# vlongle/pixie

Hardware: AMD Instinct MI355X
Metric: voxels/s (128^3 U-Net fwd) + MPM particle-steps/s (higher is better)
Workload: dtype f32 (operands split fp16 hi+lo, 3 f16 MFMAs/product, fp32 accumulate); 1 GPU; 128^3x64 feature grid -> SegmentationUNet+RegressionUNet forward (+argmax/one-hot combine), 1 scene per GPU per step; grid=128, feature_channels=64, parallelism=scene-parallel x1, executor=c+hip_graph

## Files before the change

### pixie_amd/csrc/conv3d_f16x3.hip

```cpp
#include <hip/hip_runtime.h>

#include <cstdlib>
#include <map>
#include <string>
#include <type_traits>

#include "../../include/pixie_hip.h"
#include "common.h"
#include "conv_plan.h"

namespace pixie {

typedef float f32x16 __attribute__((ext_vector_type(16)));
typedef _Float16 f16x8 __attribute__((ext_vector_type(8)));

constexpr int kW16HeaderU4 = 4;

struct Conv16Args {
    const float* in0; const float* in1;
    int c0, cin;
    int ID, IH, IW;
    int LD, LH, LW;
    int ups;
    int stride;
    int OD, OH, OW;
    const float* pro_a; const float* pro_b; const float* gamma; const float* beta;
    int act;
    const uint4* w16;
    const float* wf;
    const float* bias;
    int cout, coutp;
    const float* residual; float* out;
    const unsigned* amax0; const unsigned* amax1;
    float in_bound;
    int TX, TY, TZ, lTX, lTY;
    int tiles_x, tiles_y, tiles_z, n_tiles;
    int HX, HY, HZ, HYX, CS;
    unsigned mHX, mHYX;
    float* stats; unsigned* out_amax;
    float* partial; int chunks_per_slice;
    int epi_lds;
    const float* sk_in0; const float* sk_in1;
    int sk_c0, sk_cin;
    const uint4* sk_w16; const float* sk_bias;
    const unsigned* sk_amax0; const unsigned* sk_amax1;
};

__device__ __forceinline__ int fast_div16(int n, int d, unsigned magic) {
    return (d == 1) ? n : (int)__umulhi((unsigned)n, magic);
}
__device__ __forceinline__ float act16(float t, int act) {
    if (act == 1) return t > 0.0f ? t : 0.02f * t;
    if (act == 2) return t / (1.0f + __expf(-t));
    return t;
}
__device__ __forceinline__ float act16_staged(float t, int act) {
    if (act == 1) return fmaxf(t, 0.02f * t);
    if (act == 2) return t / (1.0f + __expf(-t));
    return t;
}
__device__ __forceinline__ int scale_exponent(float bound) {
    const unsigned bits = __float_as_uint(bound);
    const int eb = (int)((bits >> 23) & 0xffu) - 127;
    if (!(bound > 0.0f) || eb > 100) return 0;
    int e = 14 - eb;
    return e > 100 ? 100 : (e < -100 ? -100 : e);
}
__device__ __forceinline__ float pow2i(int e) { return __uint_as_float((unsigned)(e + 127) << 23); }

template <int KS, int MB, int NB, bool EX = false, bool SP = false, int SK = 0, bool PAIR = false>
__device__ __forceinline__ void conv3d_f16x3_body(const Conv16Args& A) {
    static_assert(!PAIR || (MB == 2 && !EX && !SP && SK == 0), "pair form: the plain f16x3 body with 64 c_out per quartet");
    static_assert(!SP || (KS == 3 && NB == 4 && !EX), "sub-pixel path: 3^3, two x parities x two voxel blocks per wave");
    static_assert(SK == 0 || (!EX && !SP), "folded skip (SK: 1 register-fed, 2 staged through LDS): f16x3, no sub-pixel form");
    extern __shared__ uint4 smem16[];
    constexpr int PAD = (KS == 3) ? 1 : 0;
    constexpr int NW = 4, NT = 64 * NW;
    const int bufsz = 4 * A.CS;

    const int tid = threadIdx.x;
    const int lane = tid & 63;
    const int quartet = PAIR ? __builtin_amdgcn_readfirstlane(tid >> 8) : 0;
    const int wave = PAIR ? (tid >> 6) & 3 : tid >> 6;
    const int qtid = PAIR ? tid & 255 : tid;
    const int kh = lane >> 5;
    const int l31 = lane & 31;

    int t = blockIdx.x;
    {
        const int per = (A.n_tiles + 7) >> 3;
        const int cand = (t & 7) * per + (t >> 3);
        if ((A.n_tiles & 7) == 0) t = cand;
    }
    int par = 0;
    if constexpr (SP) { par = t & 3; t >>= 2; }
    const int py = par & 1, pz = par >> 1;
    const int tx = t % A.tiles_x; t /= A.tiles_x;
    const int ty = t % A.tiles_y;
    const int tz = t / A.tiles_y;
    const int ox0 = tx * A.TX, oy0 = ty * A.TY, oz0 = tz * A.TZ;
    const int cout0 = (PAIR ? 2 * (int)blockIdx.y + quartet : (int)blockIdx.y) * (MB * 32);
    const int lx0 = SP ? ox0 - 1 : ox0 * A.stride - PAD;
    const int ly0 = SP ? oy0 - 1 + py : oy0 * A.stride - PAD;
    const int lz0 = SP ? oz0 - 1 + pz : oz0 * A.stride - PAD;
    const size_t ISP = (size_t)A.ID * A.IH * A.IW;
    const size_t OSP = (size_t)A.OD * A.OH * A.OW;

    int voff[NB];
    int ovox[NB];
    bool valid[NB];
#pragma unroll
    for (int nb = 0; nb < NB; ++nb) {
        if constexpr (SP) {
            const int px = nb >> 1;
            const int j = (wave * 2 + (nb & 1)) * 32 + l31;
            int x = j & (A.TX - 1);
            int y = (j >> A.lTX) & (A.TY - 1);
            int z = j >> (A.lTX + A.lTY);
            const int gx = 2 * (ox0 + x) + px, gy = 2 * (oy0 + y) + py, gz = 2 * (oz0 + z) + pz;
            const bool v = (z < A.TZ) && (gx < A.OW) && (gy < A.OH) && (gz < A.OD);
            if (!v) { x = 0; y = 0; z = 0; }
            voff[nb] = (z * A.HY + y) * A.HX + x + px + kh * A.CS;
            ovox[nb] = v ? (gz * A.OH + gy) * A.OW + gx : 0;
            valid[nb] = v;
            continue;
        }
        const int j = (wave * NB + nb) * 32 + l31;
        int x = j & (A.TX - 1);
        int y = (j >> A.lTX) & (A.TY - 1);
        int z = j >> (A.lTX + A.lTY);
        const bool v = (z < A.TZ) && (ox0 + x < A.OW) && (oy0 + y < A.OH) && (oz0 + z < A.OD);
        if (!v) { x = 0; y = 0; z = 0; }
        voff[nb] = ((z * A.HY + y) * A.HX + x) * A.stride + kh * A.CS;
        ovox[nb] = ((oz0 + z) * A.OH + (oy0 + y)) * A.OW + ox0 + x;
        valid[nb] = v;
    }

    float bound = A.in_bound;
    if (A.amax0) {
        bound = __uint_as_float(*A.amax0);
        if (A.amax1) bound = fmaxf(bound, __uint_as_float(*A.amax1));
    }
    const int ex = EX ? 0 : scale_exponent(bound);
    const float sx = pow2i(ex);

    f32x16 acc[MB][NB];
#pragma unroll
    for (int mb = 0; mb < MB; ++mb)
#pragma unroll
        for (int nb = 0; nb < NB; ++nb)
#pragma unroll
            for (int r = 0; r < 16; ++r) acc[mb][nb][r] = 0.0f;

    const int KG = A.cin >> 3;
    const size_t tap_stride = (size_t)KG * A.coutp;
    const size_t plane = (size_t)(SP ? 64 : KS * KS * KS) * tap_stride;
    const uint4* wHi = A.w16 + kW16HeaderU4 + (size_t)kh * A.coutp + cout0 + l31 + (size_t)(par * 16) * tap_stride;
    const uint4* wLo = wHi + plane;
    const float* wF = A.wf + (size_t)kh * A.coutp + cout0 + l31;

    constexpr int TAPS = KS * KS * KS;
    auto stage_chunk = [&](int c_base, uint4* buf, int stid, int nthr, int s0, int s1) {
        uint4* bHi = buf;
        uint4* bLo = buf + 2 * A.CS;
        float pa[16], pb[16];
        {
            float pv = 0.0f;
            if (A.pro_a) pv = (lane & 16) ? A.pro_b[c_base + (lane & 15)] : A.pro_a[c_base + (lane & 15)];
#pragma unroll
            for (int j = 0; j < 16; ++j) {
                pa[j] = __int_as_float(__builtin_amdgcn_readlane(__float_as_int(pv), j));
                pb[j] = __int_as_float(__builtin_amdgcn_readlane(__float_as_int(pv), 16 + j));
            }
        }
        const bool has_aff = A.gamma != nullptr;
        using T = std::true_type; using F = std::false_type;
        if constexpr (EX) {
            float* bF = reinterpret_cast<float*>(buf);
            for (int v0 = stid; v0 < A.CS; v0 += 2 * nthr) {
                float val[2][16];
                float gm[2], bt[2];
                int sidx[2];
                bool ok[2];
#pragma unroll
                for (int u = 0; u < 2; ++u) {
                    const int vox = v0 + u * nthr;
                    int rem = vox;
                    const int hz = fast_div16(rem, A.HYX, A.mHYX);
                    rem -= hz * A.HYX;
                    const int hy = fast_div16(rem, A.HX, A.mHX);
                    const int hx = rem - hy * A.HX;
                    const int lz = lz0 + hz, ly = ly0 + hy, lx = lx0 + hx;
                    ok[u] = vox < A.CS && (unsigned)lz < (unsigned)A.LD && (unsigned)ly < (unsigned)A.LH && (unsigned)lx < (unsigned)A.LW;
                    sidx[u] = ok[u] ? ((lz >> A.ups) * A.IH + (ly >> A.ups)) * A.IW + (lx >> A.ups) : 0;
                }
#pragma unroll
                for (int u = 0; u < 2; ++u) {
#pragma unroll
                    for (int j = 0; j < 16; ++j) {
                        const int cg = c_base + j;
                        const float* src = (cg < A.c0) ? (A.in0 + (size_t)cg * ISP) : (A.in1 + (size_t)(cg - A.c0) * ISP);
                        val[u][j] = src[sidx[u]];
                    }
                    gm[u] = 1.0f; bt[u] = 0.0f;
                    if (has_aff) { gm[u] = A.gamma[sidx[u]]; bt[u] = A.beta[sidx[u]]; }
// ... 185 lines not shown
        const uint4* ldsLo = buf + 2 * A.CS;
        const uint4* wh = wHi + (size_t)(c_base >> 3) * A.coutp;
        const uint4* wl = wLo + (size_t)(c_base >> 3) * A.coutp;
        if constexpr (SP) {
            f16x8 ah[MB], al[MB];
#pragma unroll
            for (int mb = 0; mb < MB; ++mb) {
                ah[mb] = __builtin_bit_cast(f16x8, wh[mb * 32]);
                al[mb] = __builtin_bit_cast(f16x8, wl[mb * 32]);
            }
#pragma unroll 1
            for (int zy = 0; zy < 4; ++zy) {
                const int rowoff = ((zy >> 1) * A.HY + (zy & 1)) * A.HX;
                const int zyn = zy < 3 ? zy + 1 : 3;
#pragma unroll
                for (int q = 0; q < 4; ++q) {
                    const int ex = q >> 1, px = q & 1;
                    const size_t nxt = (q < 3) ? (size_t)(((q + 1) & 1) * 8 + zy * 2 + ((q + 1) >> 1)) * tap_stride : (size_t)(zyn * 2) * tap_stride;
                    f16x8 ahn[MB], aln[MB];
#pragma unroll
                    for (int mb = 0; mb < MB; ++mb) {
                        ahn[mb] = __builtin_bit_cast(f16x8, wh[nxt + mb * 32]);
                        aln[mb] = __builtin_bit_cast(f16x8, wl[nxt + mb * 32]);
                    }
                    __builtin_amdgcn_sched_barrier(0);
                    f16x8 bh[2], bl[2];
#pragma unroll
                    for (int s = 0; s < 2; ++s) {
                        bh[s] = __builtin_bit_cast(f16x8, ldsHi[voff[px * 2 + s] + rowoff + ex]);
                        bl[s] = __builtin_bit_cast(f16x8, ldsLo[voff[px * 2 + s] + rowoff + ex]);
                    }
#pragma unroll
                    for (int mb = 0; mb < MB; ++mb)
#pragma unroll
                        for (int s = 0; s < 2; ++s)
                            acc[mb][px * 2 + s] = __builtin_amdgcn_mfma_f32_32x32x16_f16(al[mb], bh[s], acc[mb][px * 2 + s], 0, 0, 0);
#pragma unroll
                    for (int mb = 0; mb < MB; ++mb)
#pragma unroll
                        for (int s = 0; s < 2; ++s)
                            acc[mb][px * 2 + s] = __builtin_amdgcn_mfma_f32_32x32x16_f16(ah[mb], bl[s], acc[mb][px * 2 + s], 0, 0, 0);
#pragma unroll
                    for (int mb = 0; mb < MB; ++mb)
#pragma unroll
                        for (int s = 0; s < 2; ++s)
                            acc[mb][px * 2 + s] = __builtin_amdgcn_mfma_f32_32x32x16_f16(ah[mb], bh[s], acc[mb][px * 2 + s], 0, 0, 0);
#pragma unroll
                    for (int mb = 0; mb < MB; ++mb) { ah[mb] = ahn[mb]; al[mb] = aln[mb]; }
                }
            }
            __builtin_amdgcn_s_setprio(0);
            return;
        }
        f16x8 ah[MB], al[MB];
#pragma unroll
        for (int mb = 0; mb < MB; ++mb) {
            ah[mb] = __builtin_bit_cast(f16x8, wh[mb * 32]);
            al[mb] = __builtin_bit_cast(f16x8, wl[mb * 32]);
        }
#pragma unroll 1
        for (int zy = 0; zy < KS * KS; ++zy) {
            const int dz = zy / KS, dy = zy - dz * KS;
            const int rowoff = (dz * A.HY + dy) * A.HX;
#pragma unroll
            for (int dx = 0; dx < KS; ++dx) {
                const int tap = zy * KS + dx;
                const int nxt = (tap + 1 < TAPS) ? tap + 1 : tap;
                f16x8 ahn[MB], aln[MB];
#pragma unroll
                for (int mb = 0; mb < MB; ++mb) {
                    ahn[mb] = __builtin_bit_cast(f16x8, wh[(size_t)nxt * tap_stride + mb * 32]);
                    aln[mb] = __builtin_bit_cast(f16x8, wl[(size_t)nxt * tap_stride + mb * 32]);
                }
                __builtin_amdgcn_sched_barrier(0);
                f16x8 bh[NB], bl[NB];
#pragma unroll
                for (int nb = 0; nb < NB; ++nb) {
                    bh[nb] = __builtin_bit_cast(f16x8, ldsHi[voff[nb] + rowoff + dx]);
                    bl[nb] = __builtin_bit_cast(f16x8, ldsLo[voff[nb] + rowoff + dx]);
                }
#pragma unroll
                for (int mb = 0; mb < MB; ++mb)
#pragma unroll
                    for (int nb = 0; nb < NB; ++nb)
                        acc[mb][nb] = __builtin_amdgcn_mfma_f32_32x32x16_f16(al[mb], bh[nb], acc[mb][nb], 0, 0, 0);
#pragma unroll
                for (int mb = 0; mb < MB; ++mb)
#pragma unroll
                    for (int nb = 0; nb < NB; ++nb)
                        acc[mb][nb] = __builtin_amdgcn_mfma_f32_32x32x16_f16(ah[mb], bl[nb], acc[mb][nb], 0, 0, 0);
#pragma unroll
                for (int mb = 0; mb < MB; ++mb)
#pragma unroll
                    for (int nb = 0; nb < NB; ++nb)
                        acc[mb][nb] = __builtin_amdgcn_mfma_f32_32x32x16_f16(ah[mb], bh[nb], acc[mb][nb], 0, 0, 0);
#pragma unroll
                for (int mb = 0; mb < MB; ++mb) { ah[mb] = ahn[mb]; al[mb] = aln[mb]; }
            }
        }
        __builtin_amdgcn_s_setprio(0);
    };

    float inv2 = 0.0f;
    {
        const int c_begin = A.partial ? (int)blockIdx.z * A.chunks_per_slice * 16 : 0;
        const int c_end = A.partial ? min(A.cin, c_begin + A.chunks_per_slice * 16) : A.cin;
        if constexpr (PAIR) {
            const int n_chunks = (c_end - c_begin) >> 4;
            const int half = (A.CS + 1) >> 1;
            const int s0 = quartet ? half : 0, s1 = quartet ? A.CS : half;
#pragma unroll 1
            for (int h = -1; h < 2 * n_chunks; ++h) {
                const int k = h >> 1;
                const bool stage = (h < 0 || ((h + quartet) & 1) == 0) && k + 1 < n_chunks;
                const bool multiply = h >= 0 && ((h + quartet) & 1) != 0;
                if (stage) stage_chunk(c_begin + 16 * (k + 1), smem16 + ((k + 1) & 1) * bufsz, qtid, NT, s0, s1);
                if (multiply) mfma_chunk(c_begin + 16 * k, smem16 + (k & 1) * bufsz);
                if (h & 1) __syncthreads();
            }
        } else {
        for (int c_base = c_begin; c_base < c_end; c_base += 16) {
            __syncthreads();
            stage_chunk(c_base, smem16, tid, NT, 0, A.CS);
            __syncthreads();
            mfma_chunk(c_base, smem16);
        }
        }
        if constexpr (SK != 0) {
            float sb = __uint_as_float(*A.sk_amax0);
            if (A.sk_amax1) sb = fmaxf(sb, __uint_as_float(*A.sk_amax1));
            const int ex2 = scale_exponent(sb);
            const float sx2 = pow2i(ex2);
            const float inv_main = __uint_as_float(A.w16[0].x) * pow2i(-ex);
            inv2 = __uint_as_float(A.sk_w16[0].x) * pow2i(-ex2);
            const float ratio = inv_main / inv2;
#pragma unroll
            for (int mb = 0; mb < MB; ++mb)
#pragma unroll
                for (int nb = 0; nb < NB; ++nb)
#pragma unroll
                    for (int r = 0; r < 16; ++r) acc[mb][nb][r] *= ratio;
            auto sk_chunks = [&]() {
                int l31s = l31, khs = kh, waves = wave;
                asm volatile("" : "+v"(l31s), "+v"(khs), "+v"(waves));
                const unsigned chb = 4u * (unsigned)ISP;
                unsigned off[NB];
#pragma unroll
                for (int nb = 0; nb < NB; ++nb) {
                    const int j = (waves * NB + nb) * 32 + l31s;
                    const int x = j & (A.TX - 1), y = (j >> A.lTX) & (A.TY - 1), z = j >> (A.lTX + A.lTY);
                    off[nb] = (valid[nb] ? 4u * (unsigned)(((oz0 + z) * A.IH + (oy0 + y)) * A.IW + ox0 + x) : 0u) + 8u * (unsigned)khs * chb;
// ... 68 lines not shown
                        const bool okv = (ox0 + x < A.OW) && (oy0 + y < A.OH) && (oz0 + z < A.OD);
                        const size_t sidx = okv ? ((size_t)(oz0 + z) * A.IH + (oy0 + y)) * A.IW + ox0 + x : 0;
                        float val[16];
#pragma unroll
                        for (int q = 0; q < 16; ++q) {
                            const int cg = c2 + q;
                            const float* src = (cg < A.sk_c0) ? (A.sk_in0 + (size_t)cg * ISP) : (A.sk_in1 + (size_t)(cg - A.sk_c0) * ISP);
                            val[q] = src[sidx];
                        }
                        f16x8 vh[2], vl[2];
#pragma unroll
                        for (int q = 0; q < 16; ++q) {
                            const float sc = okv ? val[q] * sx2 : 0.0f;
                            const _Float16 hq = (_Float16)sc;
                            vh[q >> 3][q & 7] = hq;
                            vl[q >> 3][q & 7] = (_Float16)(sc - (float)hq);
                        }
                        const int slot = (z * A.HY + y) * A.HX + x + centre;
                        bHi[slot] = __builtin_bit_cast(uint4, vh[0]);
                        bHi[A.CS + slot] = __builtin_bit_cast(uint4, vh[1]);
                        bLo[slot] = __builtin_bit_cast(uint4, vl[0]);
                        bLo[A.CS + slot] = __builtin_bit_cast(uint4, vl[1]);
                    }
                    __syncthreads();
                    f16x8 bh[NB], bl[NB];
#pragma unroll
                    for (int nb = 0; nb < NB; ++nb) {
                        bh[nb] = __builtin_bit_cast(f16x8, bHi[voff[nb] + centre]);
                        bl[nb] = __builtin_bit_cast(f16x8, bLo[voff[nb] + centre]);
                    }
#pragma unroll
                    for (int mb = 0; mb < MB; ++mb)
#pragma unroll
                        for (int nb = 0; nb < NB; ++nb)
                            acc[mb][nb] = __builtin_amdgcn_mfma_f32_32x32x16_f16(al[mb], bh[nb], acc[mb][nb], 0, 0, 0);
#pragma unroll
                    for (int mb = 0; mb < MB; ++mb)
#pragma unroll
                        for (int nb = 0; nb < NB; ++nb)
                            acc[mb][nb] = __builtin_amdgcn_mfma_f32_32x32x16_f16(ah[mb], bl[nb], acc[mb][nb], 0, 0, 0);
#pragma unroll
                    for (int mb = 0; mb < MB; ++mb)
#pragma unroll
                        for (int nb = 0; nb < NB; ++nb)
                            acc[mb][nb] = __builtin_amdgcn_mfma_f32_32x32x16_f16(ah[mb], bh[nb], acc[mb][nb], 0, 0, 0);
                }
            } else {
                sk_chunks();
            }
        }
    }

    const float inv = EX ? 1.0f : (SK != 0 ? inv2 : __uint_as_float(A.w16[0].x) * pow2i(-ex));
    if (A.partial) {
        float* dst = A.partial + (size_t)blockIdx.z * A.cout * OSP;
#pragma unroll
        for (int mb = 0; mb < MB; ++mb)
#pragma unroll
            for (int r = 0; r < 16; ++r) {
                const int co = cout0 + mb * 32 + (r & 3) + 8 * (r >> 2) + 4 * kh;
                if (co < A.cout) {
#pragma unroll
                    for (int nb = 0; nb < NB; ++nb)
                        if (valid[nb]) dst[(size_t)co * OSP + ovox[nb]] = acc[mb][nb][r] * inv;
                }
            }
        return;
    }
    constexpr int LDO_ = NB * 32 + 4;
    float* red = reinterpret_cast<float*>(smem16) + (PAIR ? (A.epi_lds ? 2 * NW * 32 * LDO_ : 0) + quartet * (NW * MB * 64) : 0);
    float wmax = 0.0f;
    const bool full = SP ? (A.epi_lds && cout0 + MB * 32 <= A.cout && (A.TX & 1) == 0 && (A.OW & 3) == 0 && NW * 64 <= A.TX * A.TY * A.TZ &&
                            2 * (ox0 + A.TX) <= A.OW && 2 * (oy0 + A.TY) <= A.OH && 2 * (oz0 + A.TZ) <= A.OD)
                         : (A.epi_lds && cout0 + MB * 32 <= A.cout && (A.TX & 3) == 0 && (A.OW & 3) == 0 && NW * NB * 32 <= A.TX * A.TY * A.TZ &&
                            ox0 + A.TX <= A.OW && oy0 + A.TY <= A.OH && oz0 + A.TZ <= A.OD);
    if (full) {
        constexpr int LDO = NB * 32 + 4;
        float* ldsO = reinterpret_cast<float*>(smem16) + (quartet * NW + wave) * (32 * LDO);
        if constexpr (!PAIR) red = reinterpret_cast<float*>(smem16) + NW * 32 * LDO;
        constexpr int LPR = NB * 8;
        constexpr int RPI = 32 / LPR;
        constexpr int NIT = 16 / RPI;
        constexpr int G = 4;
        constexpr int GPB = NIT / G;
        constexpr int NGRP = MB * GPB;
        const int rsub = l31 / LPR, colq = 4 * (l31 % LPR), nbq = colq >> 5;
        const float* nobias = EX ? A.wf : reinterpret_cast<const float*>(A.w16);
        const bool hb0 = A.bias != nullptr, hb1 = A.sk_bias != nullptr;
        float braw[MB][2];
#pragma unroll
        for (int mb = 0; mb < MB; ++mb) {
            braw[mb][0] = (hb0 ? A.bias : nobias)[cout0 + mb * 32 + l31];
            braw[mb][1] = (hb1 ? A.sk_bias : nobias)[cout0 + mb * 32 + l31];
        }
        __syncthreads();
        const int jq = SP ? wave * 64 + (colq >> 1) : (wave * NB + nbq) * 32 + (colq & 31);
        const int xq = jq & (A.TX - 1), yq = (jq >> A.lTX) & (A.TY - 1), zq = jq >> (A.lTX + A.lTY);
        const size_t ovq = SP ? ((size_t)(2 * (oz0 + zq) + pz) * A.OH + (2 * (oy0 + yq) + py)) * A.OW + 2 * (ox0 + xq)
                              : ((size_t)(oz0 + zq) * A.OH + (oy0 + yq)) * A.OW + ox0 + xq;
        const size_t orow0 = (size_t)(cout0 + kh * RPI + rsub) * OSP + ovq;
        auto rows = [&](auto res_c, auto stats_c) {
            constexpr bool RES = decltype(res_c)::value, STATS = decltype(stats_c)::value;
            size_t step = (size_t)(2 * RPI) * OSP;
            asm volatile("" : "+s"(step));
            const float* pr = A.residual + orow0;
            float* po = A.out + orow0;
            float4 r4[2][G];
            auto fetch = [&](int q) {
#pragma unroll
                for (int g = 0; g < G; ++g) { r4[q & 1][g] = *reinterpret_cast<const float4*>(pr); pr += step; }
            };
#pragma unroll
            for (int q = 0; q < NGRP; ++q) {
                const int mb = q / GPB, it0 = (q % GPB) * G;
                asm volatile("" ::: "memory");
                if (q % GPB == 0) {
                    const int brow = __float_as_int((hb0 ? braw[mb][0] : 0.0f) + (hb1 ? braw[mb][1] : 0.0f));
#pragma unroll
                    for (int r = 0; r < 16; ++r) {
                        const int row = (r & 3) + 8 * (r >> 2);
                        const int blo = __builtin_amdgcn_readlane(brow, row), bhi = __builtin_amdgcn_readlane(brow, row + 4);
                        const float bv = __int_as_float(kh ? bhi : blo);
#pragma unroll
                        for (int nb = 0; nb < NB; ++nb)
                            ldsO[((r & 3) + 8 * (r >> 2) + 4 * kh) * LDO + (SP ? 2 * ((nb & 1) * 32 + l31) + (nb >> 1) : nb * 32 + l31)] =
                                __builtin_fmaf(acc[mb][nb][r], inv, bv);
                    }
                }
                if constexpr (RES) {
                    if (q == 0) fetch(0);
                    if (q + 1 < NGRP) fetch(q + 1);
                }
                float4 v4[G];
#pragma unroll
                for (int g = 0; g < G; ++g) {
                    const int rowl = (2 * (it0 + g) + kh) * RPI + rsub;
                    v4[g] = *reinterpret_cast<const float4*>(ldsO + rowl * LDO + colq);
                    if constexpr (RES) { v4[g].x += r4[q & 1][g].x; v4[g].y += r4[q & 1][g].y; v4[g].z += r4[q & 1][g].z; v4[g].w += r4[q & 1][g].w; }
                    *reinterpret_cast<float4*>(po) = v4[g]; po += step;
                }
                if constexpr (STATS) {
                    float s1[G], s2[G];
#pragma unroll
                    for (int g = 0; g < G; ++g) {
                        const float4 v = v4[g];
                        s1[g] = (v.x + v.y) + (v.z + v.w);
                        s2[g] = (v.x * v.x + v.y * v.y) + (v.z * v.z + v.w * v.w);
                        wmax = fmaxf(fmaxf(wmax, fmaxf(fabsf(v.x), fabsf(v.y))), fmaxf(fabsf(v.z), fabsf(v.w)));
                    }
                    asm volatile("" : "+v"(wmax));
#pragma unroll
                    for (int off = LPR / 2; off > 0; off >>= 1) {
                        float t1[G], t2[G];
#pragma unroll
                        for (int g = 0; g < G; ++g) { t1[g] = __shfl_xor(s1[g], off, 64); t2[g] = __shfl_xor(s2[g], off, 64); }
#pragma unroll
                        for (int g = 0; g < G; ++g) { s1[g] += t1[g]; s2[g] += t2[g]; }
                    }
                    if ((l31 % LPR) == 0) {
#pragma unroll
                        for (int g = 0; g < G; ++g) {
                            const int rowl = (2 * (it0 + g) + kh) * RPI + rsub;
                            red[(wave * MB * 32 + mb * 32 + rowl) * 2] = s1[g]; red[(wave * MB * 32 + mb * 32 + rowl) * 2 + 1] = s2[g];
                        }
                    }
                }
            }
        };
        using T = std::true_type; using F = std::false_type;
        if (A.residual) { if (A.stats) rows(T{}, T{}); else rows(T{}, F{}); }
        else { if (A.stats) rows(F{}, T{}); else rows(F{}, F{}); }
    } else {
    if (PAIR || A.stats) __syncthreads();
#pragma unroll
    for (int mb = 0; mb < MB; ++mb) {
#pragma unroll
        for (int r = 0; r < 16; ++r) {
            const int row = mb * 32 + (r & 3) + 8 * (r >> 2) + 4 * kh;
            const int co = cout0 + row;
            float s1 = 0.0f, s2 = 0.0f;
            if (co < A.cout) {
                const float bv = (A.bias ? A.bias[co] : 0.0f) + (A.sk_bias ? A.sk_bias[co] : 0.0f);
#pragma unroll
                for (int nb = 0; nb < NB; ++nb) {
                    if (valid[nb]) {
                        const size_t o = (size_t)co * OSP + ovox[nb];
                        float val = acc[mb][nb][r] * inv + bv;
                        if (A.residual) val += A.residual[o];
                        A.out[o] = val;
                        s1 += val; s2 += val * val; wmax = fmaxf(wmax, fabsf(val));
                    }
                }
            }
            if (A.stats) {
#pragma unroll
                for (int off = 16; off > 0; off >>= 1) { s1 += __shfl_xor(s1, off, 64); s2 += __shfl_xor(s2, off, 64); }
                if (l31 == 0) { red[(wave * MB * 32 + row) * 2] = s1; red[(wave * MB * 32 + row) * 2 + 1] = s2; }
            }
        }
    }
    }
    if (A.stats) {
        __syncthreads();
        if (qtid < MB * 32 * 2) {
            float t = red[qtid];
#pragma unroll
            for (int w = 1; w < NW; ++w) t += red[w * MB * 64 + qtid];
            A.stats[((size_t)blockIdx.x * A.coutp + cout0) * 2 + qtid] = t;
        }
        if (A.out_amax) {
#pragma unroll
            for (int off = 32; off > 0; off >>= 1) wmax = fmaxf(wmax, __shfl_xor(wmax, off, 64));
            if (lane == 0 && wmax > 0.0f) atomicMax(A.out_amax, __float_as_uint(wmax));
        }
    }
}

template <int KS, int MB, int NB>
__global__ __launch_bounds__(256, 2) void conv3d_f16x3_kernel(Conv16Args A) {
    conv3d_f16x3_body<KS, MB, NB>(A);
}
template <int KS, int NB>
__global__ __launch_bounds__(512, 1) void conv3d_f16x3_pair_kernel(Conv16Args A) {
    conv3d_f16x3_body<KS, 2, NB, false, false, 0, true>(A);
}
template <int KS, int MB, int NB, bool STAGED>
__global__ __launch_bounds__(256, 2) void conv3d_f16x3_skip_kernel(Conv16Args A) {
    conv3d_f16x3_body<KS, MB, NB, false, false, STAGED ? 2 : 1>(A);
}
template <int KS, int MB, int NB>
__global__ __launch_bounds__(256, 2) void conv3d_exact_kernel(Conv16Args A) {
    conv3d_f16x3_body<KS, MB, NB, true>(A);
}
template <int MB>
__global__ __launch_bounds__(256, 2) void conv3d_f16x3_subpixel_kernel(Conv16Args A) {
    conv3d_f16x3_body<3, MB, 4, false, true>(A);
}
__global__ __launch_bounds__(256, 2) void conv3d_f16x3_c64_fullres_kernel(Conv16Args A) {
    conv3d_f16x3_body<3, 2, 4>(A);
}

struct StatParts { const void* p; int n; long cstride, tstride; int f64; };

__device__ inline void block_channel_sums(const StatParts& P, int c, double* r, double& o1, double& o2) {
    double s1 = 0.0, s2 = 0.0;
    for (int t = threadIdx.x; t < P.n; t += 256) {
        const size_t k = ((size_t)c * P.cstride + (size_t)t * P.tstride) * 2;
        if (P.f64) { const double2 v = *reinterpret_cast<const double2*>(static_cast<const double*>(P.p) + k); s1 += v.x; s2 += v.y; }
        else { const float2 v = *reinterpret_cast<const float2*>(static_cast<const float*>(P.p) + k); s1 += v.x; s2 += v.y; }
    }
    for (int off = 32; off > 0; off >>= 1) { s1 += __shfl_down(s1, off, 64); s2 += __shfl_down(s2, off, 64); }
    if ((threadIdx.x & 63) == 0) { r[2 * (threadIdx.x >> 6)] = s1; r[2 * (threadIdx.x >> 6) + 1] = s2; }
    __syncthreads();
    o1 = r[0] + r[2] + r[4] + r[6]; o2 = r[1] + r[3] + r[5] + r[7];
    __syncthreads();
}

__global__ __launch_bounds__(256) void stats_finalize_kernel(StatParts P, double* __restrict__ sums) {
    const int c = blockIdx.x;
    __shared__ double r[8];
    double s1, s2;
    block_channel_sums(P, c, r, s1, s2);
    if (threadIdx.x == 0) { sums[2 * c] = s1; sums[2 * c + 1] = s2; }
}

__global__ __launch_bounds__(256) void stats_norm_finalize_kernel(StatParts P0, double* sums0, int c0, StatParts P1, double* sums1, int channels,
                                                                  double spatial, int mode, int groups, double eps,
                                                                  const float* __restrict__ weight, const float* __restrict__ bias,
                                                                  float* __restrict__ a, float* __restrict__ b) {
    __shared__ double r[8];
    const int cpg = mode == 0 ? 1 : channels / groups;
    const int first = blockIdx.x * cpg;
    double s1 = 0.0, s2 = 0.0;
    for (int k = first; k < first + cpg; ++k) {
        const bool in0 = k < c0;
        const StatParts& P = in0 ? P0 : P1;
        double* sums = in0 ? sums0 : sums1;
        const int kc = in0 ? k : k - c0;
        double t1, t2;
        if (P.n > 0) {
            block_channel_sums(P, kc, r, t1, t2);
            if (threadIdx.x == 0) { sums[2 * kc] = t1; sums[2 * kc + 1] = t2; }
        } else {
            t1 = sums[2 * kc]; t2 = sums[2 * kc + 1];
        }
        s1 += t1; s2 += t2;
    }
    const double cnt = mode == 0 ? spatial : spatial * cpg;
    const double mean = s1 / cnt;
    double var = s2 / cnt - mean * mean;
    if (var < 0.0) var = 0.0;
    const double rstd = 1.0 / sqrt(var + eps);
    for (int k = first + threadIdx.x; k < first + cpg; k += 256) {
// ... 246 lines not shown
        const long wgs = (long)p.n_tiles * ((p.coutp + p.MB * 32 - 1) / (p.MB * 32));
        while (p.slices * 2 <= smax && wgs * p.slices < 512) p.slices *= 2;
    } else {
        const long ovol = (long)p.OD * p.OH * p.OW;
        int MB = (p.coutp >= 64) ? 2 : 1;
        int NB = (s.stride == 2) ? 1 : 4;
        auto n_wg = [&](int mb, int nb) {
            const long tiles = (ovol + 128L * nb - 1) / (128L * nb);
            return tiles * ((p.coutp + mb * 32 - 1) / (mb * 32));
        };
        int slices = 1;
        if (smax >= 2 && n_wg(MB, NB) < 512) {
            bool found = false;
            for (int nb = NB; nb >= 1 && !found; nb /= 2) {
                for (int sl = 1; sl <= smax; sl *= 2)
                    if (n_wg(MB, nb) * sl >= 512) { NB = nb; slices = sl; found = true; break; }
            }
            if (!found) { NB = 1; slices = 1; while (slices * 2 <= smax) slices *= 2; }
        } else {
            while (n_wg(MB, NB) < 512 && NB > 1) NB /= 2;
            if (n_wg(MB, NB) < 512 && MB > 1) MB = 1;
        }
        p.MB = MB; p.NB = NB; p.slices = slices;
        tile(p.OD, p.OH, p.OW, 128 * NB);
        p.HX = (p.TX - 1) * s.stride + s.ksize; p.HY = (p.TY - 1) * s.stride + s.ksize; p.HZ = (p.TZ - 1) * s.stride + s.ksize;
    }
    p.HYX = p.HY * p.HX; p.CS = p.HZ * p.HYX;
    p.mHX = magic_of(p.HX); p.mHYX = magic_of(p.HYX);
    if (p.slices > 1) p.chunks_per_slice = (chunks + p.slices - 1) / p.slices;
    p.lds_bytes = (size_t)4 * p.CS * sizeof(uint4);
    if (p.lds_bytes > 160 * 1024) return refuse(CONV_BAD_LDS);
    const size_t epi_bytes = ((size_t)4 * 32 * (p.NB * 32 + 4) + (size_t)4 * p.MB * 32 * 2) * sizeof(float);
    if (p.slices == 1 && epi_bytes <= 80 * 1024) { p.epi_lds = 1; p.lds_bytes = std::max(p.lds_bytes, epi_bytes); }
    p.grid = dim3((unsigned)p.n_tiles, (unsigned)((p.coutp + p.MB * 32 - 1) / (p.MB * 32)), (unsigned)p.slices);
    if (!p.f16x3()) return p;
    const long osp = (long)p.OD * p.OH * p.OW;
    if (p.slices > 1) {
        const int n = reduce_segments(osp);
        p.stats = ConvStatLayout{n, n, 1, 1};
        p.stats_floats = (int64_t)s.c_out * n * 2 * (int64_t)(sizeof(double) / sizeof(float));
        p.workspace_bytes = (int64_t)p.slices * s.c_out * osp * (int64_t)sizeof(float);
    } else {
        p.stats = ConvStatLayout{p.n_tiles, 1, p.coutp, 0};
        p.stats_floats = (int64_t)p.n_tiles * p.coutp * 2;
    }
    p.fullres = !sub && p.slices == 1 && s.ksize == 3 && p.MB == 2 && p.NB == 4 && cin == 64 && s.c_out == 64 && s.stride == 1 && !s.upsample &&
                s.c1 == 0 && !s.skip && osp >= 128L * 128 * 128;
    const int scin = s.skip_c0 + s.skip_c1;
    p.skip_foldable = !sub && s.stride == 1 && !s.upsample && scin > 0 && scin % 16 == 0 && s.skip_c0 % 8 == 0 && p.slices == 1;
    return p;
}

using ConvKernel = void (*)(Conv16Args);
static ConvKernel conv16_kernel(const ConvPlan& p, bool skip = false, int skip_c0 = 0) {
    if (p.path == CONV_F16X3_SUBPIXEL) return p.MB == 2 ? conv3d_f16x3_subpixel_kernel<2> : conv3d_f16x3_subpixel_kernel<1>;
    if (p.fullres) return conv3d_f16x3_c64_fullres_kernel;
#define PX_CONV16_PICK(KS_, MB_, NB_)                                                                \
    if (p.KS == KS_ && p.MB == MB_ && p.NB == NB_)                                                   \
        return p.path == CONV_EXACT_TILED ? conv3d_exact_kernel<KS_, MB_, NB_>                       \
                                          : (!skip ? conv3d_f16x3_kernel<KS_, MB_, NB_>                                \
                                                   : ((skip_c0 & 8) ? conv3d_f16x3_skip_kernel<KS_, MB_, NB_, true> : conv3d_f16x3_skip_kernel<KS_, MB_, NB_, false>));
    PX_CONV_VARIANTS(PX_CONV16_PICK)
#undef PX_CONV16_PICK
    return nullptr;
}

#ifdef PIXIE_DIAG
static int g_conv_keep_four_wave = 0;
#endif
static size_t conv_pair_lds(const ConvPlan& p, bool skip) {
#ifdef PIXIE_DIAG
    if (g_conv_keep_four_wave) return 0;
#endif
    if (p.path != CONV_F16X3 || p.fullres || skip || p.MB != 2 || p.NB != 4 || p.slices != 1 || p.coutp % 128 != 0) return 0;
    const size_t tiles = (size_t)2 * 4 * p.CS * sizeof(uint4);
    const size_t red = (size_t)2 * 4 * p.MB * 32 * 2 * sizeof(float);
    const size_t epi = p.epi_lds ? (size_t)8 * 32 * (p.NB * 32 + 4) * sizeof(float) + red : red;
    const size_t lds = std::max(tiles, epi);
    return lds <= 160 * 1024 ? lds : 0;
}
static ConvKernel conv16_pair_kernel(const ConvPlan& p) {
#define PX_CONV16_PAIR(KS_, NB_) \
    if (p.KS == KS_ && p.NB == NB_) return conv3d_f16x3_pair_kernel<KS_, NB_>;
    PX_CONV16_PAIR(3, 4) PX_CONV16_PAIR(1, 4)
#undef PX_CONV16_PAIR
    return nullptr;
}

static int launch(ConvKernel kern, const ConvPlan& p, const Conv16Args& a, hipStream_t st, size_t pair_lds = 0) {
    PX_REQUIRE(kern != nullptr, "conv: no kernel variant for ksize=%d MB=%d NB=%d", p.KS, p.MB, p.NB);
    PX_CHECK_HIP(allow_max_dynamic_lds(reinterpret_cast<const void*>(kern)));
    if (pair_lds) hipLaunchKernelGGL(kern, dim3(p.grid.x, p.grid.y / 2, 1), dim3(512), pair_lds, st, a);
    else hipLaunchKernelGGL(kern, p.grid, dim3(256), p.lds_bytes, st, a);
    PX_CHECK_HIP(hipGetLastError());
    return 0;
}

static Conv16Args conv16_args(const pixie_conv_desc* d, const ConvPlan& p) {
    Conv16Args a{};
    a.in0 = d->d_in0; a.in1 = d->d_in1; a.c0 = d->c0; a.cin = d->c0 + d->c1;
    a.ID = d->in_d; a.IH = d->in_h; a.IW = d->in_w;
    a.LD = p.LD; a.LH = p.LH; a.LW = p.LW; a.ups = p.ups; a.stride = d->stride;
    a.OD = p.OD; a.OH = p.OH; a.OW = p.OW;
    a.pro_a = d->d_pro_a; a.pro_b = d->d_pro_b; a.gamma = d->d_gamma; a.beta = d->d_beta; a.act = d->act;
    a.bias = d->d_bias; a.cout = d->c_out; a.coutp = p.coutp;
    a.residual = d->d_residual; a.out = d->d_out;
    a.TX = p.TX; a.TY = p.TY; a.TZ = p.TZ; a.lTX = p.lTX; a.lTY = p.lTY;
    a.tiles_x = p.tiles_x; a.tiles_y = p.tiles_y; a.tiles_z = p.tiles_z; a.n_tiles = p.n_tiles;
    a.HX = p.HX; a.HY = p.HY; a.HZ = p.HZ; a.HYX = p.HYX; a.CS = p.CS; a.mHX = p.mHX; a.mHYX = p.mHYX;
    a.chunks_per_slice = p.chunks_per_slice; a.epi_lds = p.epi_lds;
    return a;
}

int conv3d_f16x3_forward(const pixie_conv_desc* d, const ConvPlan& p, hipStream_t st) {
    PX_REQUIRE(p.refusal != CONV_BAD_STRIDE, "f16x3 conv: stride must be 1, or 2 for a 3^3 kernel");
    PX_REQUIRE(p.refusal != CONV_BAD_CHANNELS, "f16x3 conv: c_in must be a multiple of 16 (got %d+%d)", d->c0, d->c1);
    PX_REQUIRE(d->d_in_amax0 != nullptr || d->in_bound > 0.0f, "f16x3 conv: needs d_in_amax0 or a positive in_bound");
    PX_REQUIRE(d->c1 == 0 || d->d_in_amax0 == nullptr || d->d_in_amax1 != nullptr, "f16x3 conv: second input needs its own amax slot");
    PX_REQUIRE(p.refusal != CONV_BAD_SUBPIXEL, "f16x3 conv: sub-pixel weights need upsample = 1, ksize = 3, stride = 1 and no folded skip");
    PX_REQUIRE((int64_t)d->in_d * d->in_h * d->in_w * 16 * (int64_t)sizeof(float) < (int64_t)1 << 32, "f16x3 conv: 16 channels of the input must span less than 4 GiB");
    Conv16Args a = conv16_args(d, p);
    a.w16 = reinterpret_cast<const uint4*>(d->d_w16);
    a.amax0 = d->d_in_amax0; a.amax1 = (d->c1 > 0) ? d->d_in_amax1 : nullptr; a.in_bound = d->in_bound;
    a.stats = d->d_out_stats; a.out_amax = d->d_out_amax;
    if (d->d_skip_w16) {
        PX_REQUIRE(p.skip_foldable, "f16x3 conv: this launch cannot fold a skip convolution (pixie_conv_skip_foldable)");
        PX_REQUIRE(d->d_skip_in0 && d->d_skip_amax0 && (d->skip_c1 == 0 || (d->d_skip_in1 && d->d_skip_amax1)), "f16x3 conv: folded skip needs its inputs and their amax slots");
        PX_REQUIRE((int64_t)d->in_d * d->in_h * d->in_w * 16 * (int64_t)sizeof(float) < (int64_t)1 << 32, "f16x3 conv: folded skip: 16 channels of the skip input must span less than 4 GiB");
        a.sk_in0 = d->d_skip_in0; a.sk_in1 = d->d_skip_in1; a.sk_c0 = d->skip_c0; a.sk_cin = d->skip_c0 + d->skip_c1;
        a.sk_w16 = reinterpret_cast<const uint4*>(d->d_skip_w16); a.sk_bias = d->d_skip_bias;
        a.sk_amax0 = d->d_skip_amax0; a.sk_amax1 = d->skip_c1 > 0 ? d->d_skip_amax1 : nullptr;
    }
    if (p.slices > 1) {
        a.partial = static_cast<float*>(d->d_workspace);
        a.stats = nullptr; a.out_amax = nullptr;
    }
    PX_REQUIRE(p.refusal != CONV_BAD_LDS, "f16x3 conv: tile needs %zu B of LDS", p.lds_bytes);
    PX_REQUIRE(p.f16x3(), "f16x3 conv: bad sizes");
    const size_t pair_lds = conv_pair_lds(p, a.sk_w16 != nullptr);
    if (int rc = launch(pair_lds ? conv16_pair_kernel(p) : conv16_kernel(p, a.sk_w16 != nullptr, a.sk_c0), p, a, st, pair_lds)) return rc;
    if (p.slices == 1) return 0;
    const long osp = (long)a.OD * a.OH * a.OW, n_elems = (long)a.cout * osp;
    if (d->d_out_stats) {
        const dim3 rgrid((unsigned)reduce_segments(osp), (unsigned)a.cout);
        double* rstats = reinterpret_cast<double*>(d->d_out_stats);
        PX_REQUIRE((reinterpret_cast<size_t>(rstats) & 7) == 0, "f16x3 conv: d_out_stats of a split-K launch must be 8-byte aligned");
        const bool vec = osp % 4 == 0 && ((reinterpret_cast<size_t>(a.partial) | reinterpret_cast<size_t>(a.residual) | reinterpret_cast<size_t>(a.out)) & 15) == 0;
        if (vec) hipLaunchKernelGGL(splitk_reduce_stats_kernel<true>, rgrid, dim3(256), 0, st, a.partial, p.slices, n_elems, osp, a.bias, a.residual,
                                    a.out, rstats, d->d_out_amax);
        else hipLaunchKernelGGL(splitk_reduce_stats_kernel<false>, rgrid, dim3(256), 0, st, a.partial, p.slices, n_elems, osp, a.bias, a.residual,
                                a.out, rstats, d->d_out_amax);
    } else {
        hipLaunchKernelGGL(splitk_reduce_kernel, dim3((unsigned)((n_elems + 255) / 256)), dim3(256), 0, st, a.partial, p.slices, n_elems, osp,
                           a.bias, a.residual, a.out);
    }
    PX_CHECK_HIP(hipGetLastError());
    return 0;
}

int conv3d_exact_forward(const pixie_conv_desc* d, const ConvPlan& p, hipStream_t st) {
    PX_REQUIRE(p.refusal != CONV_BAD_LDS, "exact conv: tile needs %zu B of LDS", p.lds_bytes);
    PX_REQUIRE(p.path == CONV_EXACT_TILED, "exact conv: bad sizes");
    Conv16Args a = conv16_args(d, p);
    a.wf = d->d_w;
    a.in_bound = 1.0f;
    return launch(conv16_kernel(p), p, a, st);
}

}

using namespace pixie;

static ConvPlan plan_of(const pixie_conv_desc* d) { return d ? conv_plan(conv_shape_of(d)) : ConvPlan{}; }
static StatParts stat_parts(const ConvPlan& p, const void* stats) { return StatParts{stats, p.stats.n, p.stats.cstride, p.stats.tstride, p.stats.f64}; }

extern "C" int64_t pixie_conv_stats_floats(const pixie_conv_desc* d) { return plan_of(d).stats_floats; }

extern "C" int64_t pixie_conv_workspace_bytes(const pixie_conv_desc* d) {
    if (!d) return 0;
    ConvShape s = conv_shape_of(d);
    s.workspace = true;
    return conv_plan(s).workspace_bytes;
}

#ifdef PIXIE_DIAG
extern "C" int pixie_conv_kernel_variant(const pixie_conv_desc* d, int* slices_out) {
    if (!d) {
        const int before = g_conv_keep_four_wave;
        if (slices_out && (*slices_out == 0 || *slices_out == 1)) g_conv_keep_four_wave = *slices_out;
        return before;
    }
    const ConvPlan p = plan_of(d);
    if (slices_out) *slices_out = p.f16x3() ? p.slices : 1;
    if (!p.f16x3()) return 0;
    if (p.path == CONV_F16X3_SUBPIXEL) return 8300 + p.MB * 10 + p.NB;
    if (p.fullres) return 9324;
    return p.KS * 100 + p.MB * 10 + p.NB;
}

extern "C" int pixie_conv_tile_geometry(const pixie_conv_desc* d, int32_t out[10]) {
    const ConvPlan p = plan_of(d);
    if (!out && d) return (int)conv_pair_lds(p, d->d_skip_w16 != nullptr);
    if (!out || !p.tiled()) return 1;
    const int32_t v[10] = {p.TX, p.TY, p.TZ, p.tiles_x, p.tiles_y, p.tiles_z, p.epi_lds, p.slices, p.MB, p.NB};
    for (int i = 0; i < 10; ++i) out[i] = v[i];
    return 0;
}

extern "C" int pixie_conv_stats_layout(const pixie_conv_desc* d, int64_t out[6]) {
    const ConvPlan p = plan_of(d);
    if (!out || !p.f16x3()) return 1;
    out[0] = p.stats.n; out[1] = p.stats.cstride; out[2] = p.stats.tstride; out[3] = p.stats.f64; out[4] = p.stats.f64 ? kReduceSeg : 0;
    out[5] = p.coutp;
    return 0;
}
#endif

extern "C" int pixie_conv_skip_foldable(const pixie_conv_desc* d) { return plan_of(d).skip_foldable ? 1 : 0; }

extern "C" int pixie_stats_finalize(const float* d_stats, const pixie_conv_desc* d, double* d_sums, void* stream) {
    PX_REQUIRE(d_stats && d && d_sums, "pixie_stats_finalize: null argument");
    hipLaunchKernelGGL(stats_finalize_kernel, dim3((unsigned)d->c_out), dim3(256), 0, as_stream(stream), stat_parts(plan_of(d), d_stats), d_sums);
    PX_CHECK_HIP(hipGetLastError());
    return 0;
}

extern "C" int pixie_stats_norm_finalize(const float* d_stats0, const pixie_conv_desc* desc0, double* d_sums0, const float* d_stats1,
                                         const pixie_conv_desc* desc1, double* d_sums1, int c1, int64_t spatial, int mode, int groups,
                                         double eps, const float* d_weight, const float* d_bias, float* d_a, float* d_b, void* stream) {
    PX_REQUIRE(desc0 && d_sums0 && d_a && d_b && spatial > 0 && c1 >= 0, "pixie_stats_norm_finalize: bad arguments");
    PX_REQUIRE(c1 == 0 || d_sums1, "pixie_stats_norm_finalize: a second part needs d_sums1");
    PX_REQUIRE(!d_stats1 || desc1, "pixie_stats_norm_finalize: d_stats1 needs its descriptor");
    const int c0 = desc0->c_out, channels = c0 + c1;
    PX_REQUIRE(!d_stats1 || desc1->c_out == c1, "pixie_stats_norm_finalize: desc1 has %d output channels, c1 is %d", desc1 ? desc1->c_out : 0, c1);
    PX_REQUIRE(mode == 0 || (mode == 1 && groups > 0 && channels % groups == 0), "pixie_stats_norm_finalize: bad mode/groups");
    const StatParts none{nullptr, 0, 0, 0, 0};
    const StatParts p0 = d_stats0 ? stat_parts(plan_of(desc0), d_stats0) : none;
    const StatParts p1 = d_stats1 ? stat_parts(plan_of(desc1), d_stats1) : none;
    hipLaunchKernelGGL(stats_norm_finalize_kernel, dim3((unsigned)(mode == 0 ? channels : groups)), dim3(256), 0, as_stream(stream), p0, d_sums0, c0,
                       p1, d_sums1, channels, (double)spatial, mode, groups, eps, d_weight, d_bias, d_a, d_b);
    PX_CHECK_HIP(hipGetLastError());
    return 0;
// ... 54 lines not shown
```

Baseline: 27.61 million voxels/s.

## Use 16x16x32 MFMA tap loop with buffer-loaded weights for 3^3 convs

```diff
diff --git a/pixie_amd/csrc/conv3d_f16x3.hip b/pixie_amd/csrc/conv3d_f16x3.hip
--- a/pixie_amd/csrc/conv3d_f16x3.hip
+++ b/pixie_amd/csrc/conv3d_f16x3.hip
@@ -12,6 +12,7 @@
 namespace pixie {
 
 typedef float f32x16 __attribute__((ext_vector_type(16)));
+typedef float f32x4 __attribute__((ext_vector_type(4)));
 typedef _Float16 f16x8 __attribute__((ext_vector_type(8)));
 
 constexpr int kW16HeaderU4 = 4;
@@ -68,9 +69,10 @@
 }
 __device__ __forceinline__ float pow2i(int e) { return __uint_as_float((unsigned)(e + 127) << 23); }
 
-template <int KS, int MB, int NB, bool EX = false, bool SP = false, int SK = 0, bool PAIR = false>
+template <int KS, int MB, int NB, bool EX = false, bool SP = false, int SK = 0, bool PAIR = false, bool N16 = false>
 __device__ __forceinline__ void conv3d_f16x3_body(const Conv16Args& A) {
     static_assert(!PAIR || (MB == 2 && !EX && !SP && SK == 0), "pair form: the plain f16x3 body with 64 c_out per quartet");
+    static_assert(!N16 || (KS == 3 && MB == 2 && NB == 4 && !EX && !SP && SK == 0), "16x16x32 tap loop: <3,2,4>, plain f16x3");
     static_assert(!SP || (KS == 3 && NB == 4 && !EX), "sub-pixel path: 3^3, two x parities x two voxel blocks per wave");
     static_assert(SK == 0 || (!EX && !SP), "folded skip (SK: 1 register-fed, 2 staged through LDS): f16x3, no sub-pixel form");
     extern __shared__ uint4 smem16[];
@@ -85,6 +87,7 @@
     const int qtid = PAIR ? tid & 255 : tid;
     const int kh = lane >> 5;
     const int l31 = lane & 31;
+    const int c16 = lane & 15, kg = (lane >> 4) & 1, q16 = lane >> 4;
 
     int t = blockIdx.x;
     {
@@ -125,13 +128,13 @@
             valid[nb] = v;
             continue;
         }
-        const int j = (wave * NB + nb) * 32 + l31;
+        const int j = (wave * NB + nb) * 32 + (N16 ? c16 : l31);
         int x = j & (A.TX - 1);
         int y = (j >> A.lTX) & (A.TY - 1);
         int z = j >> (A.lTX + A.lTY);
         const bool v = (z < A.TZ) && (ox0 + x < A.OW) && (oy0 + y < A.OH) && (oz0 + z < A.OD);
         if (!v) { x = 0; y = 0; z = 0; }
-        voff[nb] = ((z * A.HY + y) * A.HX + x) * A.stride + kh * A.CS;
+        voff[nb] = ((z * A.HY + y) * A.HX + x) * A.stride + (N16 ? kg : kh) * A.CS;
         ovox[nb] = ((oz0 + z) * A.OH + (oy0 + y)) * A.OW + ox0 + x;
         valid[nb] = v;
     }
@@ -144,13 +147,14 @@
     const int ex = EX ? 0 : scale_exponent(bound);
     const float sx = pow2i(ex);
 
-    f32x16 acc[MB][NB];
-#pragma unroll
-    for (int mb = 0; mb < MB; ++mb)
-#pragma unroll
-        for (int nb = 0; nb < NB; ++nb)
-#pragma unroll
-            for (int r = 0; r < 16; ++r) acc[mb][nb][r] = 0.0f;
+    constexpr int AM = N16 ? 4 : MB, AN = N16 ? 8 : NB, AR = N16 ? 4 : 16;
+    std::conditional_t<N16, f32x4, f32x16> acc[AM][AN];
+#pragma unroll
+    for (int mb = 0; mb < AM; ++mb)
+#pragma unroll
+        for (int nb = 0; nb < AN; ++nb)
+#pragma unroll
+            for (int r = 0; r < AR; ++r) acc[mb][nb][r] = 0.0f;
 
     const int KG = A.cin >> 3;
     const size_t tap_stride = (size_t)KG * A.coutp;
@@ -442,6 +446,65 @@
             __builtin_amdgcn_s_setprio(0);
             return;
         }
+        if constexpr (N16) {
+            const uint4* wrow = A.w16 + kW16HeaderU4 + (size_t)(c_base >> 3) * A.coutp + cout0;
+            const __amdgpu_buffer_rsrc_t rh = __builtin_amdgcn_make_buffer_rsrc(const_cast<uint4*>(wrow), 0, 0x40000000, 0x00020000);
+            const __amdgpu_buffer_rsrc_t rl = __builtin_amdgcn_make_buffer_rsrc(const_cast<uint4*>(wrow + plane), 0, 0x40000000, 0x00020000);
+            const unsigned ts16 = 16u * (unsigned)tap_stride;
+            const bool up = lane >= 32;
+            const unsigned aoff = 16u * (unsigned)(kg * A.coutp + c16) + (up ? ts16 : 0u);
+            const unsigned aoff1 = up ? 0x80000000u : aoff;
+            typedef unsigned u32x4 __attribute__((ext_vector_type(4)));
+            auto load_a = [&](f16x8 (&h)[4], f16x8 (&l)[4], unsigned lane_off, unsigned tap_off) {
+#pragma unroll
+                for (int m = 0; m < 4; ++m) {
+                    h[m] = __builtin_bit_cast(f16x8, (u32x4)__builtin_amdgcn_raw_buffer_load_b128(rh, (int)(lane_off + 256u * m), (int)tap_off, 0));
+                    l[m] = __builtin_bit_cast(f16x8, (u32x4)__builtin_amdgcn_raw_buffer_load_b128(rl, (int)(lane_off + 256u * m), (int)tap_off, 0));
+                }
+            };
+            int offa = 0, dx = 0, dy = 0;
+            auto next_tap = [&](int off) {
+                ++off;
+                if (++dx == 3) { dx = 0; off += A.HX - 3; if (++dy == 3) { dy = 0; off += (A.HY - 3) * A.HX; } }
+                return off;
+            };
+            f16x8 ah[4], al[4];
+            load_a(ah, al, aoff, 0u);
+            int offb = next_tap(offa);
+            int offl = up ? offb : offa;
+            f16x8 bh = __builtin_bit_cast(f16x8, ldsHi[voff[0] + offl]);
+            f16x8 bl = __builtin_bit_cast(f16x8, ldsLo[voff[0] + offl]);
+#pragma unroll 1
+            for (int s = 0; s < 14; ++s) {
+                const int sn = s < 13 ? s + 1 : 13;
+                f16x8 ahn[4], aln[4];
+                load_a(ahn, aln, sn == 13 ? aoff1 : aoff, (unsigned)(2 * sn) * ts16);
+                __builtin_amdgcn_sched_barrier(0);
+                int offl_n = offl;
+                if (s < 13) {
+                    offa = next_tap(offb);
+                    offb = s < 12 ? next_tap(offa) : offa;
+                    offl_n = up ? offb : offa;
+                }
+#pragma unroll
+                for (int n = 0; n < 8; ++n) {
+                    const int vn = n < 7 ? voff[(n + 1) >> 1] + offl + 16 * ((n + 1) & 1) : voff[0] + offl_n;
+                    const f16x8 bhn = __builtin_bit_cast(f16x8, ldsHi[vn]);
+                    const f16x8 bln = __builtin_bit_cast(f16x8, ldsLo[vn]);
+                    __builtin_amdgcn_sched_barrier(0);
+#pragma unroll
+                    for (int m = 0; m < 4; ++m) acc[m][n] = __builtin_amdgcn_mfma_f32_16x16x32_f16(al[m], bh, acc[m][n], 0, 0, 0);
+#pragma unroll
+                    for (int m = 0; m < 4; ++m) acc[m][n] = __builtin_amdgcn_mfma_f32_16x16x32_f16(ah[m], bl, acc[m][n], 0, 0, 0);
+#pragma unroll
+                    for (int m = 0; m < 4; ++m) acc[m][n] = __builtin_amdgcn_mfma_f32_16x16x32_f16(ah[m], bh, acc[m][n], 0, 0, 0);
+                    bh = bhn; bl = bln;
+                }
+#pragma unroll
+                for (int m = 0; m < 4; ++m) { ah[m] = ahn[m]; al[m] = aln[m]; }
+                offl = offl_n;
+            }
+        } else {
         f16x8 ah[MB], al[MB];
 #pragma unroll
         for (int mb = 0; mb < MB; ++mb) {
@@ -487,6 +550,7 @@
 #pragma unroll
                 for (int mb = 0; mb < MB; ++mb) { ah[mb] = ahn[mb]; al[mb] = aln[mb]; }
             }
+        }
         }
         __builtin_amdgcn_s_setprio(0);
     };
@@ -661,8 +725,33 @@
     }
 
     const float inv = EX ? 1.0f : (SK != 0 ? inv2 : __uint_as_float(A.w16[0].x) * pow2i(-ex));
+    int c16e = c16, wavee = wave;
+    if constexpr (N16) asm volatile("" : "+v"(c16e), "+v"(wavee));
+    auto vox16 = [&](int n, bool& v) {
+        const int j = (wavee * NB + (n >> 1)) * 32 + 16 * (n & 1) + c16e;
+        const int x = j & (A.TX - 1), y = (j >> A.lTX) & (A.TY - 1), z = j >> (A.lTX + A.lTY);
+        v = (z < A.TZ) && (ox0 + x < A.OW) && (oy0 + y < A.OH) && (oz0 + z < A.OD);
+        return v ? ((oz0 + z) * A.OH + (oy0 + y)) * A.OW + ox0 + x : 0;
+    };
     if (A.partial) {
         float* dst = A.partial + (size_t)blockIdx.z * A.cout * OSP;
+        if constexpr (N16) {
+            int ov[8]; bool vv[8];
+#pragma unroll
+            for (int n = 0; n < 8; ++n) ov[n] = vox16(n, vv[n]);
+#pragma unroll
+            for (int m = 0; m < 4; ++m)
+#pragma unroll
+                for (int r = 0; r < 4; ++r) {
+                    const int co = cout0 + 16 * m + 4 * q16 + r;
+                    if (co < A.cout) {
+#pragma unroll
+                        for (int n = 0; n < 8; ++n)
+                            if (vv[n]) dst[(size_t)co * OSP + ov[n]] = acc[m][n][r] * inv;
+                    }
+                }
+            return;
+        } else {
 #pragma unroll
         for (int mb = 0; mb < MB; ++mb)
 #pragma unroll
@@ -675,6 +764,7 @@
                 }
             }
         return;
+        }
     }
     constexpr int LDO_ = NB * 32 + 4;
     float* red = reinterpret_cast<float*>(smem16) + (PAIR ? (A.epi_lds ? 2 * NW * 32 * LDO_ : 0) + quartet * (NW * MB * 64) : 0);
@@ -723,6 +813,20 @@
             for (int q = 0; q < NGRP; ++q) {
                 const int mb = q / GPB, it0 = (q % GPB) * G;
                 asm volatile("" ::: "memory");
+                if constexpr (N16) {
+                    if (q % GPB == 0) {
+                        const float brow = (hb0 ? braw[mb][0] : 0.0f) + (hb1 ? braw[mb][1] : 0.0f);
+#pragma unroll
+                        for (int mm = 0; mm < 2; ++mm)
+#pragma unroll
+                            for (int r = 0; r < 4; ++r) {
+                                const float bv = __shfl(brow, 16 * mm + 4 * q16 + r, 64);
+#pragma unroll
+                                for (int n = 0; n < 8; ++n)
+                                    ldsO[(16 * mm + 4 * q16 + r) * LDO + 16 * n + c16] = __builtin_fmaf(acc[2 * mb + mm][n][r], inv, bv);
+                            }
+                    }
+                } else
                 if (q % GPB == 0) {
                     const int brow = __float_as_int((hb0 ? braw[mb][0] : 0.0f) + (hb1 ? braw[mb][1] : 0.0f));
 #pragma unroll
@@ -781,6 +885,38 @@
         else { if (A.stats) rows(F{}, T{}); else rows(F{}, F{}); }
     } else {
     if (PAIR || A.stats) __syncthreads();
+    if constexpr (N16) {
+        int ov[8]; bool vv[8];
+#pragma unroll
+        for (int n = 0; n < 8; ++n) ov[n] = vox16(n, vv[n]);
+#pragma unroll
+        for (int m = 0; m < 4; ++m) {
+#pragma unroll
+            for (int r = 0; r < 4; ++r) {
+                const int row = 16 * m + 4 * q16 + r;
+                const int co = cout0 + row;
+                float s1 = 0.0f, s2 = 0.0f;
+                if (co < A.cout) {
+                    const float bv = A.bias ? A.bias[co] : 0.0f;
+#pragma unroll
+                    for (int n = 0; n < 8; ++n) {
+                        if (vv[n]) {
+                            const size_t o = (size_t)co * OSP + ov[n];
+                            float val = acc[m][n][r] * inv + bv;
+                            if (A.residual) val += A.residual[o];
+                            A.out[o] = val;
+                            s1 += val; s2 += val * val; wmax = fmaxf(wmax, fabsf(val));
+                        }
+                    }
+                }
+                if (A.stats) {
+#pragma unroll
+                    for (int off = 8; off > 0; off >>= 1) { s1 += __shfl_xor(s1, off, 64); s2 += __shfl_xor(s2, off, 64); }
+                    if (c16 == 0) { red[(wave * MB * 32 + row) * 2] = s1; red[(wave * MB * 32 + row) * 2 + 1] = s2; }
+                }
+            }
+        }
+    } else {
 #pragma unroll
     for (int mb = 0; mb < MB; ++mb) {
 #pragma unroll
@@ -809,6 +945,7 @@
         }
     }
     }
+    }
     if (A.stats) {
         __syncthreads();
         if (qtid < MB * 32 * 2) {
@@ -846,8 +983,19 @@
     conv3d_f16x3_body<3, MB, 4, false, true>(A);
 }
 __global__ __launch_bounds__(256, 2) void conv3d_f16x3_c64_fullres_kernel(Conv16Args A) {
+    conv3d_f16x3_body<3, 2, 4, false, false, 0, false, true>(A);
+}
+__global__ __launch_bounds__(256, 2) void conv3d_f16x3_n16_kernel(Conv16Args A) {
+    conv3d_f16x3_body<3, 2, 4, false, false, 0, false, true>(A);
+}
+__global__ __launch_bounds__(512, 1) void conv3d_f16x3_n16_pair_kernel(Conv16Args A) {
+    conv3d_f16x3_body<3, 2, 4, false, false, 0, true, true>(A);
+}
+#ifdef PIXIE_DIAG
+__global__ __launch_bounds__(256, 2) void conv3d_f16x3_c64_fullres_m32_kernel(Conv16Args A) {
     conv3d_f16x3_body<3, 2, 4>(A);
 }
+#endif
 
 struct StatParts { const void* p; int n; long cstride, tstride; int f64; };
 
@@ -1200,9 +1348,23 @@
 }
 
 using ConvKernel = void (*)(Conv16Args);
-static ConvKernel conv16_kernel(const ConvPlan& p, bool skip = false, int skip_c0 = 0) {
+#ifdef PIXIE_DIAG
+static int g_conv_keep_m32 = 0;
+#endif
+static bool conv_n16(const ConvPlan& p, bool skip, int cin) {
+#ifdef PIXIE_DIAG
+    if (g_conv_keep_m32) return false;
+#endif
+    return p.path == CONV_F16X3 && !skip && p.KS == 3 && p.MB == 2 && p.NB == 4 && p.TX == 32 && p.HX == 34 && cin != 32 &&
+           (int64_t)2 * 27 * (cin / 8) * p.coutp * 16 < (int64_t)0x40000000;
+}
+static ConvKernel conv16_kernel(const ConvPlan& p, bool skip = false, int skip_c0 = 0, int cin = 0) {
     if (p.path == CONV_F16X3_SUBPIXEL) return p.MB == 2 ? conv3d_f16x3_subpixel_kernel<2> : conv3d_f16x3_subpixel_kernel<1>;
+#ifdef PIXIE_DIAG
+    if (p.fullres && !conv_n16(p, skip, cin)) return conv3d_f16x3_c64_fullres_m32_kernel;
+#endif
     if (p.fullres) return conv3d_f16x3_c64_fullres_kernel;
+    if (conv_n16(p, skip, cin)) return conv3d_f16x3_n16_kernel;
 #define PX_CONV16_PICK(KS_, MB_, NB_)                                                                \
     if (p.KS == KS_ && p.MB == MB_ && p.NB == NB_)                                                   \
         return p.path == CONV_EXACT_TILED ? conv3d_exact_kernel<KS_, MB_, NB_>                       \
@@ -1227,7 +1389,8 @@
     const size_t lds = std::max(tiles, epi);
     return lds <= 160 * 1024 ? lds : 0;
 }
-static ConvKernel conv16_pair_kernel(const ConvPlan& p) {
+static ConvKernel conv16_pair_kernel(const ConvPlan& p, int cin) {
+    if (conv_n16(p, false, cin)) return conv3d_f16x3_n16_pair_kernel;
 #define PX_CONV16_PAIR(KS_, NB_) \
     if (p.KS == KS_ && p.NB == NB_) return conv3d_f16x3_pair_kernel<KS_, NB_>;
     PX_CONV16_PAIR(3, 4) PX_CONV16_PAIR(1, 4)
@@ -1286,7 +1449,7 @@
     PX_REQUIRE(p.refusal != CONV_BAD_LDS, "f16x3 conv: tile needs %zu B of LDS", p.lds_bytes);
     PX_REQUIRE(p.f16x3(), "f16x3 conv: bad sizes");
     const size_t pair_lds = conv_pair_lds(p, a.sk_w16 != nullptr);
-    if (int rc = launch(pair_lds ? conv16_pair_kernel(p) : conv16_kernel(p, a.sk_w16 != nullptr, a.sk_c0), p, a, st, pair_lds)) return rc;
+    if (int rc = launch(pair_lds ? conv16_pair_kernel(p, a.cin) : conv16_kernel(p, a.sk_w16 != nullptr, a.sk_c0, a.cin), p, a, st, pair_lds)) return rc;
     if (p.slices == 1) return 0;
     const long osp = (long)a.OD * a.OH * a.OW, n_elems = (long)a.cout * osp;
     if (d->d_out_stats) {
@@ -1334,8 +1497,8 @@
 #ifdef PIXIE_DIAG
 extern "C" int pixie_conv_kernel_variant(const pixie_conv_desc* d, int* slices_out) {
     if (!d) {
-        const int before = g_conv_keep_four_wave;
-        if (slices_out && (*slices_out == 0 || *slices_out == 1)) g_conv_keep_four_wave = *slices_out;
+        const int before = g_conv_keep_four_wave | (g_conv_keep_m32 << 1);
+        if (slices_out && *slices_out >= 0 && *slices_out <= 3) { g_conv_keep_four_wave = *slices_out & 1; g_conv_keep_m32 = (*slices_out >> 1) & 1; }
         return before;
     }
     const ConvPlan p = plan_of(d);
```

Result: no change. 27.72 million voxels/s (median of 3 runs) (+0.4%).
